# jhamrick/gaussian_processes

Measured on AMD Instinct MI355X. Metric: GP fit+predict wall-clock (kernel build + Cholesky + solve + log_lh + posterior mean), lower is better.
Workload: dtype f64; 1 GPU; N=65536 d=32 RBF(GaussianKernel) f64, m=1000 test points, h=1 w=0.5*sqrt(d) s=1; N=65536, d=32, m=1000, parallelism=1 GPU

## Files before the change

gaussian_processes_amd/_lib.py:

```python
import ctypes
import os
from ctypes import (POINTER, c_char_p, c_double, c_float, c_int, c_int64, c_size_t,
                    c_uint64, c_void_p)

import numpy as np

_HERE = os.path.dirname(os.path.abspath(__file__))
LIB_PATH = os.path.join(_HERE, "libgpx.so")

OK = 0
ERR_ARG, ERR_HIP, ERR_NO_DEVICE, ERR_NOMEM, ERR_UNSUPPORTED, ERR_INTERNAL = -1, -2, -3, -4, -5, -6
(ROUTE_TRSV_OPS, ROUTE_TRSV_STEPS, ROUTE_PANEL_RES, ROUTE_PANEL_CHAIN, ROUTE_FIT_RIDE, ROUTE_FIT_TWO_SOLVES,
 ROUTE_GEMM_FAST, ROUTE_GEMM_GENERIC, ROUTE_SYRK_EXACT, ROUTE_SYRK_PATCH, ROUTE_MG_BCAST_ONE, ROUTE_MG_BCAST_SAG,
 ROUTE_FIT_OPS_AHEAD, ROUTE_TRSM_OPS, ROUTE_POTRF_PAIR, ROUTE_VAR_CHUNK, ROUTE_LOO_CHUNK, ROUTE_TRSM_L_OPS,
 ROUTE_GRAD_CHUNK, ROUTE_EXTEND, ROUTE_SAMPLE, ROUTE_KAPPLY_FUSED, ROUTE_KAPPLY_GEMM, ROUTE_PATHS_GRAD_CHUNK) = range(24)
PROF_RANDN, PROF_RFF, PROF_KAPPLY, PROF_KAPPLY_GRAD = 14, 15, 16, 17
F64, F32 = 0, 1
KERNEL_GAUSSIAN, KERNEL_PERIODIC, KERNEL_GAUSSIAN_ARD = 0, 1, 2
ARD_MAX_D = 64
FULL, LOWER = 0, 1
(K, DK_DH, DK_DW, DK_DP, D2K_DHDH, D2K_DHDW, D2K_DHDP, D2K_DWDW, D2K_DWDP, D2K_DPDP) = range(10)
MIN_LOG = -705.6238298100243

MEMBER_BY_NAME = {
    "K": K, "dK_dh": DK_DH, "dK_dw": DK_DW, "dK_dp": DK_DP,
    "d2K_dhdh": D2K_DHDH, "d2K_dhdw": D2K_DHDW, "d2K_dwdh": D2K_DHDW,
    "d2K_dhdp": D2K_DHDP, "d2K_dpdh": D2K_DHDP, "d2K_dwdw": D2K_DWDW,
    "d2K_dwdp": D2K_DWDP, "d2K_dpdw": D2K_DWDP, "d2K_dpdp": D2K_DPDP,
}

# ... 103 lines not shown
    "gpx_gp_extend_from_K": (c_int, [c_void_p, c_double_p, c_double_p, c_int64, c_double_p, c_double_p, POINTER(c_void_p),
                                     c_int_p]),
    "gpx_gp_sample": (c_int, [c_void_p, c_double_p, c_int64, c_int64, c_uint64, c_int, c_double, c_double_p, c_int_p]),
    "gpx_gp_sample_from_K": (c_int, [c_void_p, c_double_p, c_double_p, c_int64, c_int64, c_uint64, c_int, c_double, c_double_p,
                                     c_int_p]),
    "gpx_gp_paths_create": (c_int, [c_void_p, c_int64, c_int64, c_uint64, POINTER(c_void_p)]),
    "gpx_paths_eval": (c_int, [c_void_p, c_double_p, c_int64, c_int64, c_double_p]),
    "gpx_paths_grad": (c_int, [c_void_p, c_double_p, c_int64, c_int64, c_double_p, c_double_p]),
    "gpx_paths_get": (c_int, [c_void_p, c_double_p, c_double_p, c_double_p]),
    "gpx_paths_describe": (c_int, [c_void_p, c_int_p, c_int_p, POINTER(c_int64), c_int_p, POINTER(c_int64), POINTER(c_int64),
                                   POINTER(c_uint64)]),
    "gpx_debug_paths_timing": (c_int, [c_void_p, POINTER(c_float)]),
    "gpx_paths_destroy": (c_int, [c_void_p]),
    "gpx_debug_var_plan": (c_int, [c_int, c_int64, c_int64, c_int64, c_size_t, POINTER(c_int64), POINTER(c_int64),
                                   POINTER(c_size_t)]),
    "gpx_gp_get_Kxx": (c_int, [c_void_p, c_double_p, c_int64]),
    "gpx_gp_get_Lxx": (c_int, [c_void_p, c_double_p, c_int64]),
    "gpx_gp_get_alpha": (c_int, [c_void_p, c_double_p]),
    "gpx_gp_get_inv_Kxx": (c_int, [c_void_p, c_double_p, c_int64]),
    "gpx_gp_dloglh_dtheta": (c_int, [c_void_p, c_double_p]),
    "gpx_gp_dlh_d2lh": (c_int, [c_void_p, c_double_p, c_double_p, c_double_p]),
    "gpx_gp_dm_dtheta": (c_int, [c_void_p, c_double_p, c_int64, c_double_p]),
    "gpx_gp_fit_batch": (c_int, [c_void_p, c_double_p, c_int64, c_double_p, c_int_p]),
    "gpx_gp_fit_batch_grad": (c_int, [c_void_p, c_double_p, c_int64, c_double_p, c_double_p, c_double_p, c_int_p]),
    "gpx_gp_save": (c_int, [c_void_p, c_char_p]),
    "gpx_gp_load": (c_int, [POINTER(c_void_p), c_char_p]),
    "gpx_gp_describe": (c_int, [c_void_p, c_int_p, c_int_p, POINTER(c_int64), c_int_p, c_double_p, c_double_p]),
    "gpx_gp_get_xy": (c_int, [c_void_p, c_double_p, c_double_p]),
    "gpx_gp_last_timing": (c_int, [c_void_p, POINTER(c_float)]),
    "gpx_gp_device_ptrs": (c_int, [c_void_p, POINTER(c_void_p), POINTER(c_int64), POINTER(c_void_p),
# ... 131 lines not shown
def mem_free():
    f, t = c_size_t(0), c_size_t(0)
    check(load().gpx_mem_info(ctypes.byref(f), ctypes.byref(t)))
    return int(f.value)


def var_plan(dtype_id, n, m, chunk_rows=0, free_bytes=None):
    if free_bytes is None:
        free_bytes = mem_free()
    rows, chunks, nbytes = c_int64(0), c_int64(0), c_size_t(0)
    check(load().gpx_debug_var_plan(int(dtype_id), int(n), int(m), int(chunk_rows), int(free_bytes), ctypes.byref(rows),
                                    ctypes.byref(chunks), ctypes.byref(nbytes)))
    return rows.value, chunks.value, int(nbytes.value)


def route_count(route):
    v = c_int64(0)
    check(load().gpx_debug_route_count(int(route), ctypes.byref(v)))
    return v.value


def route_reset():
    check(load().gpx_debug_route_reset())


def kapply_fused_max(value=-1):
    prev = c_int64(0)
    check(load().gpx_debug_kapply_fused_max(int(value), ctypes.byref(prev)))
    return prev.value

# ... 7 lines not shown
```

gaussian_processes_amd/csrc/gpx_common.h:

```cpp
#pragma once
#include <hip/hip_runtime.h>
#include <stdint.h>
#include <stdio.h>
#include <stdlib.h>
#include <string.h>
#include <math.h>
#include <vector>

#include "../../include/gpx.h"
#include "gpx_tune.h"

namespace gpx {

void set_error(const char *fmt, ...);
int  hip_fail(hipError_t e, const char *what, const char *file, int line);
int  ensure_device();

#define GPX_HIP(call)                                                        \
    do {                                                                     \
        hipError_t e__ = (call);                                             \
        if (e__ != hipSuccess) return gpx::hip_fail(e__, #call, __FILE__, __LINE__); \
    } while (0)

#define GPX_TRY(call)                                                        \
// ... 5 lines not shown
#define GPX_ARG(cond, msg)                                                   \
    do {                                                                     \
        if (!(cond)) { gpx::set_error("%s: %s", __func__, msg); return GPX_ERR_ARG; } \
    } while (0)

#define GPX_LAUNCH_CHECK()                                                   \
    do {                                                                     \
        hipError_t e__ = hipGetLastError();                                  \
        if (e__ != hipSuccess) return gpx::hip_fail(e__, "kernel launch", __FILE__, __LINE__); \
    } while (0)


enum Route { RT_TRSV_OPS = 0, RT_TRSV_STEPS = 1, RT_PANEL_RES = 2, RT_PANEL_CHAIN = 3, RT_FIT_RIDE = 4,
             RT_FIT_TWO_SOLVES = 5, RT_GEMM_FAST = 6, RT_GEMM_GENERIC = 7, RT_SYRK_EXACT = 8, RT_SYRK_PATCH = 9,
             RT_MG_BCAST_ONE = 10, RT_MG_BCAST_SAG = 11, RT_FIT_OPS_AHEAD = 12, RT_TRSM_OPS = 13, RT_POTRF_PAIR = 14, RT_VAR_CHUNK = 15, RT_LOO_CHUNK = 16,
             RT_TRSM_L_OPS = 17, RT_GRAD_CHUNK = 18, RT_EXTEND = 19, RT_SAMPLE = 20, RT_KAPPLY_FUSED = 21, RT_KAPPLY_GEMM = 22, RT_PATHS_GRAD_CHUNK = 23, RT_COUNT = 24 };
void route_hit(int route);

int check_internal_info(int info);

static inline hipStream_t S(void *s) { return (hipStream_t)s; }
static inline size_t esize(int dtype) { return dtype == GPX_F64 ? 8 : 4; }
static inline int64_t round_up(int64_t v, int64_t m) { return (v + m - 1) / m * m; }
static inline int64_t cdiv(int64_t a, int64_t b) { return (a + b - 1) / b; }

static inline int order(hipEvent_t e, hipStream_t from, hipStream_t to)
{
    GPX_HIP(hipEventRecord(e, from));
    GPX_HIP(hipStreamWaitEvent(to, e, 0));
    return GPX_OK;
}
struct EventPool {
// ... 96 lines not shown
constexpr int TRSV_OPS_BLOCK = 512;
static inline int64_t trsv_ops_nblocks(int64_t n) { return n / TRSV_OPS_BLOCK; }
static inline bool trsv_ops_whole_blocks(int64_t n) { return n >= TRSV_OPS_BLOCK && n % TRSV_OPS_BLOCK == 0; }
struct TrsvOps {
    GrowBuf mem;
    bool valid = false;
    int64_t built = 0;
    void invalidate() { valid = false; built = 0; }
    static TrsvOps view(void *p, size_t bytes) { TrsvOps o; o.mem.p = p; o.mem.bytes = bytes; return o; }
};
int trsv_ops_build(int dtype, const void *L, int64_t n, int64_t ldl, TrsvOps *ops, hipStream_t st);
bool trsv_ops_ahead_ok(int dtype, const void *L, int64_t n, int64_t ldl);
bool trsm_ops_ok(int dtype, const void *L, int64_t n, int64_t ldl);
size_t trsv_ops_bytes(int dtype, int64_t n);
int trsv_ops_build_upto(int dtype, const void *L, int64_t n, int64_t ldl, TrsvOps *ops, int64_t kend, hipStream_t st);
int trsv_lower(int dtype, const void *L, int64_t n, int64_t ldl, void *b, void *x, int transpose,
               hipStream_t st, const Batch *bt = nullptr,
               TrsvOps *ops = nullptr);
int trsm_right_lt(int dtype, const void *L, int64_t n, int64_t ldl, void *X, int64_t m, int64_t ldx,
                  hipStream_t st, int x_upper = 0, TrsvOps *ops = nullptr,
                  int64_t c0 = 0);
int trsm_right_l(int dtype, const void *L, int64_t n, int64_t ldl, void *X, int64_t m, int64_t ldx, hipStream_t st,
                 TrsvOps *ops = nullptr);
int pred_grad(int dtype, int kernel, const void *xo, int64_t m, const void *x, int64_t n, int d, const double *params,
              const void *alpha, const void *B, int64_t ldb, double scale, const double *col_div, double *out_dev, hipStream_t st);
int inv_from_factor(int dtype, const void *L, int64_t n, int64_t ldl, void *X, void *W, int tri, hipStream_t st,
                    TrsvOps *ops, int count = 1, int64_t sL = 0, void *group_ops = nullptr);
int logdet_chol(int dtype, const void *L, int64_t n, int64_t ldl, double *out_dev, hipStream_t st, int count = 1,
                int64_t sL = 0, int64_t so = 0);
int dot(int dtype, const void *a, const void *b, int64_t n, double *out_dev, hipStream_t st, int count = 1,
        int64_t sa = 0, int64_t sb = 0, int64_t so = 0);
int tril(int dtype, void *A, int64_t n, int64_t lda, hipStream_t st);
int var_rows(int dtype, int kernel, const void *X, int64_t rows, int64_t n, int64_t ldx, const void *xo, int d,
// ... 41 lines not shown
```

gaussian_processes_amd/csrc/gpx_gp.hip:

```cpp
#include "gpx_common.h"
#include <cmath>
#include <vector>

#include "gpx_gp_internal.h"

namespace gpx {

template <typename T>
__global__ void cvt_from_f64_2d(const double *__restrict__ src, int64_t lds, T *__restrict__ dst, int64_t ldd, int64_t rows, int64_t cols)
{
    const int64_t c = (int64_t)blockIdx.x * blockDim.x + threadIdx.x;
    if (c >= cols) return;
    for (int64_t r = blockIdx.y; r < rows; r += gridDim.y) dst[r * ldd + c] = (T)src[r * lds + c];
}

template <typename T>
__global__ void cvt_to_f64_2d(const T *__restrict__ src, int64_t lds, double *__restrict__ dst,
                              int64_t ldd, int64_t rows, int64_t cols, int lower_only)
{
    const int64_t c = (int64_t)blockIdx.x * blockDim.x + threadIdx.x;
    if (c >= cols) return;
    for (int64_t r = blockIdx.y; r < rows; r += gridDim.y) {
        const double v = (double)src[r * lds + c];
        dst[r * ldd + c] = (lower_only && c > r) ? 0.0 : v;
// ... 76 lines not shown
{
    GpScal sc;
    GPX_TRY(gp_read_scal(g, &sc));
    if (sc.info != 0) { set_error("Kxx is not positive definite (info = %d): there is no factor %s", sc.info, what_for); return GPX_ERR_ARG; }
    return GPX_OK;
}

int check_internal_info(int info)
{
    if (info >= 0) return GPX_OK;
    set_error("internal failure inside the factorisation (info = %d: a hand-off between workgroups of the resident "
              "panel kernel timed out); the factor is not valid -- this is NOT a statement about the matrix", info);
    return GPX_ERR_INTERNAL;
}

int gp_finish_fit(gpx_gp *g, bool rhs_is_row_n, int *info)
{
    const size_t es = esize(g->dtype);
    hipStream_t st = g->st;
    if (rhs_is_row_n) {
        GPX_TRY(trsv_lower(g->dtype, g->A, g->n, g->lda, (char *)g->A + (size_t)g->n * g->lda * es, g->alpha, 1, st, nullptr, &g->ops));
    } else {
        GPX_HIP(hipMemcpyAsync(g->t0, g->y, (size_t)g->n * es, hipMemcpyDeviceToDevice, st));
        GPX_TRY(trsv_lower(g->dtype, g->A, g->n, g->lda, g->t0, g->t1, 0, st, nullptr, &g->ops));
        GPX_TRY(trsv_lower(g->dtype, g->A, g->n, g->lda, g->t1, g->alpha, 1, st, nullptr, &g->ops));
    }
    GPX_HIP(hipEventRecord(g->ev[3], st));
    GPX_TRY(logdet_chol(g->dtype, g->A, g->n, g->lda, &g->scal->logdet, st));
    GPX_TRY(dot(g->dtype, g->y, g->alpha, g->n, &g->scal->yta, st));
    GPX_HIP(hipEventRecord(g->ev[4], st));
    g->fitted = true;
    if (info) {
        GPX_HIP(hipMemcpyAsync(info, &g->scal->info, sizeof(int), hipMemcpyDeviceToHost, st));
        GPX_HIP(hipStreamSynchronize(st));
        GPX_TRY(check_internal_info(*info));
    }
    return GPX_OK;
}

// ... 242 lines not shown
    GPX_ARG(cap >= 0 && (cap == 0 || params), "bad arguments");
    if (count) *count = g->nparams;
    for (int i = 0; i < g->nparams && i < cap; ++i) params[i] = g->params[i];
    return GPX_OK;
}

int gpx_gp_set_K(gpx_gp_t *g, const double *Kxx, int64_t ld)
{
    GP_ENTER(g);
    GPX_ARG(g && Kxx && ld >= g->n, "bad arguments");
    GPX_TRY(upload_f64(g->dtype, g->A, g->lda, Kxx, ld, g->n, g->n, g->st));
    g->have_K = true; gp_unfit(g);
    return GPX_OK;
}

struct OpsAhead { gpx_gp *g; int64_t group, last; };
static int ops_ahead_step(void *user, int64_t cols_done, hipEvent_t panel_done)
{
    OpsAhead *o = (OpsAhead *)user;
    gpx_gp *g = o->g;
    const int64_t ready = std::min(trsv_ops_nblocks(cols_done), o->last);
    if (ready - g->ops.built < o->group) return GPX_OK;
    GPX_HIP(hipStreamWaitEvent(g->st_ops, panel_done, 0));
    return trsv_ops_build_upto(g->dtype, g->A, g->n, g->lda, &g->ops, ready, g->st_ops);
}

int gpx_gp_fit(gpx_gp_t *g, int *info)
{
    GP_ENTER(g);
    GPX_ARG(g, "gp is NULL");
    GPX_ARG(g->have_data && (g->have_params || g->have_K),
            "set_data and set_params (or set_K) must be called before fit");
    const GpView v = gp_view(g);
    if (!g->have_K && (!g->x_finite || !kernel_values_finite(v.kernel, v.params, g->s, g->dtype))) {
        set_error("%s (%s)", NONFINITE_MSG, g->x_finite ? "kernel parameters or s" : "x");
        return GPX_ERR_ARG;
    }
    const size_t es = esize(g->dtype);
    hipStream_t st = g->st;
    GPX_HIP(hipEventRecord(g->ev[0], st));
    if (!g->have_K)
        GPX_TRY(kmat(g->dtype, v.kernel, GPX_K, v.x, g->n, v.x, g->n, g->d, v.params, g->s * g->s,
                     GPX_LOWER, g->A, g->lda, st));
    g->have_K = false;
    g->have_kii = false;
    GPX_HIP(hipEventRecord(g->ev[1], st));
    const int64_t ride_max = tune().fit_ride_max;
    const bool ride = g->n <= ride_max;
    route_hit(ride ? RT_FIT_RIDE : RT_FIT_TWO_SOLVES);
    if (ride) GPX_HIP(hipMemcpyAsync((char *)g->A + (size_t)g->n * g->lda * es, g->y, (size_t)g->n * es, hipMemcpyDeviceToDevice, st));
    g->ops.invalidate();
    const bool ahead = tune().fit_ops_ahead != 0 && g->n >= tune().fit_ops_ahead_min &&
                       trsv_ops_ahead_ok(g->dtype, g->A, g->n, g->lda);
    const int64_t nfull = trsv_ops_nblocks(g->n), tail = tune().fit_ops_tail;
    const int64_t group = std::max<int64_t>(1, std::min(nfull, nfull - tail));
    OpsAhead oa = {g, group, std::max<int64_t>(0, nfull - tail)};
    PotrfHook hook = {ops_ahead_step, &oa};
    if (ahead) {
        if (!g->st_ops) {
            int least = 0, greatest = 0;
            GPX_HIP(hipDeviceGetStreamPriorityRange(&least, &greatest));
            GPX_HIP(hipStreamCreateWithPriority(&g->st_ops, hipStreamNonBlocking, least));
            GPX_HIP(hipEventCreateWithFlags(&g->ev_ops, hipEventDisableTiming));
        }
        GPX_TRY(g->ops.mem.reserve(trsv_ops_bytes(g->dtype, g->n), st));
        GPX_TRY(order(g->ev_ops, st, g->st_ops));
    }
    GPX_TRY(potrf(g->dtype, g->A, g->n, g->lda, &g->scal->info, st, nullptr, ride ? 1 : 0, true, ahead ? &hook : nullptr));
    if (ahead) {
        GPX_TRY(order(g->ev_ops, g->st_ops, st));
        if (g->ops.built > 0) route_hit(RT_FIT_OPS_AHEAD);
    }
    GPX_HIP(hipEventRecord(g->ev[2], st));
    return gp_finish_fit(g, ride, info);
}

static int gp_scalars(gpx_gp_t *g, double *logdet, double *yta, int *info)
{
    GP_ENTER(g);
    GPX_ARG(g && g->fitted, "gp is not fitted");
    GpScal sc;
    GPX_TRY(gp_read_scal(g, &sc));
    if (logdet) *logdet = sc.logdet;
    if (yta) *yta = sc.yta;
    if (info) *info = sc.info;
    return GPX_OK;
}

int gpx_gp_log_lh(gpx_gp_t *g, double *log_lh)
// ... 296 lines not shown
    if (!g->have_kii) GPX_TRY(gp_loo_sweep(g, ch, dm, dv, dl));
    else GPX_TRY(loo_points(g->dtype, g->kii, g->y, g->alpha, n, dm, dv, dl, g->st));
    GPX_TRY(sum_f64(dl, n, ds, g->st));
    if (mean) GPX_HIP(hipMemcpyAsync(mean, dm, (size_t)n * sizeof(double), hipMemcpyDeviceToHost, g->st));
    if (var) GPX_HIP(hipMemcpyAsync(var, dv, (size_t)n * sizeof(double), hipMemcpyDeviceToHost, g->st));
    if (log_p) GPX_HIP(hipMemcpyAsync(log_p, dl, (size_t)n * sizeof(double), hipMemcpyDeviceToHost, g->st));
    if (log_p_sum) GPX_HIP(hipMemcpyAsync(log_p_sum, ds, sizeof(double), hipMemcpyDeviceToHost, g->st));
    GPX_HIP(hipStreamSynchronize(g->st));
    return GPX_OK;
}

int gpx_debug_var_plan(int dtype, int64_t n, int64_t m, int64_t chunk_rows, size_t free_bytes,
                       int64_t *rows_per_chunk, int64_t *chunks, size_t *bytes_per_chunk)
{
    return var_plan(dtype, n, m, chunk_rows, free_bytes, rows_per_chunk, chunks, bytes_per_chunk);
}

int gpx_gp_get_Kxx(gpx_gp_t *g, double *out, int64_t ld)
{
    GP_ENTER(g);
    GPX_ARG(g && g->have_data && g->have_params && out && ld >= g->n, "bad arguments");
    const size_t es = esize(g->dtype);
    DevBuf K;
    GPX_TRY(K.alloc((size_t)g->n * g->lda * es));
    const GpView v = gp_view(g);
    GPX_TRY(kmat(g->dtype, v.kernel, GPX_K, v.x, g->n, v.x, g->n, g->d, v.params, g->s * g->s,
                 GPX_FULL, K.p, g->lda, g->st));
    return download_f64(g->dtype, out, ld, K.p, g->lda, g->n, g->n, 0, g->st);
}

// ... 402 lines not shown
```

gaussian_processes_amd/csrc/gpx_gp_internal.h:

```cpp
#pragma once
#include "gpx_common.h"
#include <cstddef>

struct GpScal {
    double logdet;
    double yta;
    int x_bad, y_bad;
    int info;
    int pad;
};
static_assert(sizeof(GpScal) == 32 && offsetof(GpScal, x_bad) == 16 && offsetof(GpScal, info) == 24, "GpScal layout");

struct gpx_gp {
    int device;
    int dtype, kernel, d, nparams;
    int64_t n, lda;
    void *x, *y, *A, *alpha, *t0, *t1;
    void *xs;
    GpScal *scal;
    hipStream_t st;
    hipEvent_t ev[6];
    double params[1 + GPX_ARD_MAX_D];
    double iso[2];
    double s;
// ... 6 lines not shown
    double *kii;
    bool have_kii;
    hipStream_t st_ops;
    hipEvent_t ev_ops;
};

namespace gpx {
int gp_scan_finite(gpx_gp *g);
int upload_f64(int dtype, void *dst, int64_t ldd, const double *src, int64_t lds, int64_t rows, int64_t cols, hipStream_t st,
               DevBuf *stage = nullptr);
int download_f64(int dtype, double *dst, int64_t ldh, const void *src, int64_t lds, int64_t rows, int64_t cols, int lower_only,
                 hipStream_t st);
int gp_read_scal(gpx_gp *g, GpScal *host);
int gp_need_factor(gpx_gp *g, const char *what_for);
static inline void gp_unfit(gpx_gp *g) { g->fitted = false; g->have_kii = false; }
int gp_finish_fit(gpx_gp *g, bool rhs_is_row_n, int *info);
static inline int nparams_of(int kernel, int d) { return kernel == GPX_KERNEL_GAUSSIAN_ARD ? 1 + d : (kernel == GPX_KERNEL_PERIODIC ? 3 : 2); }
struct GpView { int kernel; const void *x; const double *params; };
static inline GpView gp_view(const gpx_gp *g)
{
    if (g->kernel == GPX_KERNEL_GAUSSIAN_ARD) return {GPX_KERNEL_GAUSSIAN, g->xs, g->iso};
    return {g->kernel, g->x, g->params};
}
int gp_rescale(gpx_gp *g);
}

#define GP_ENTER(g)                                                          \
    GPX_ARG((g) != nullptr, "gp is NULL");                                   \
    gpx::tune_refresh();                                                     \
    gpx::DeviceGuard guard__((g)->device);                                   \
    if (guard__.rc != GPX_OK) return guard__.rc;                             \
// ... 4 lines not shown
```

gaussian_processes_amd/csrc/gpx_runtime.hip:

```cpp
#include "gpx_common.h"
#include <stdarg.h>
#include <stddef.h>
#include <dlfcn.h>
#include <atomic>
#include <mutex>
#include <set>
#include <utility>
#include <vector>

namespace gpx {

static thread_local char g_err[512] = "";

void set_error(const char *fmt, ...)
{
    va_list ap;
    va_start(ap, fmt);
    vsnprintf(g_err, sizeof(g_err), fmt, ap);
    va_end(ap);
}

int hip_fail(hipError_t e, const char *what, const char *file, int line)
{
    set_error("HIP error %d (%s) in %s at %s:%d", (int)e, hipGetErrorString(e), what, file, line);
// ... 127 lines not shown
    }
    if (b) (void)hipEventRecord(b, st);
}

static void prof_clear()
{
    std::lock_guard<std::mutex> lk(g_prof_mu);
    for (auto &r : g_prof) {
        if (r.a) (void)hipEventDestroy(r.a);
        if (r.b) (void)hipEventDestroy(r.b);
    }
    g_prof.clear();
}

static std::atomic<long long> g_route[RT_COUNT];
void route_hit(int route) { if (route >= 0 && route < RT_COUNT) g_route[route].fetch_add(1, std::memory_order_relaxed); }

static std::mutex g_attr_mu;
static std::set<std::pair<const void *, int>> g_attr_done;

int set_max_lds(const void *fn, int bytes)
{
    int dev = 0;
    GPX_HIP(hipGetDevice(&dev));
    std::lock_guard<std::mutex> lk(g_attr_mu);
    const auto key = std::make_pair(fn, dev);
    if (g_attr_done.count(key)) return GPX_OK;
    GPX_HIP(hipFuncSetAttribute(fn, hipFuncAttributeMaxDynamicSharedMemorySize, bytes));
    g_attr_done.insert(key);
    return GPX_OK;
}
// ... 330 lines not shown
```

gaussian_processes_amd/csrc/gpx_solve.hip:

```cpp
#include "gpx_common.h"
#include "gpx_kernels_dev.h"
#include "gpx_leaf.h"

namespace gpx {

constexpr int SB = 64;
constexpr int OB = TRSV_OPS_BLOCK;

template <typename T>
__global__ __launch_bounds__(256) void inv64_kernel(const T *__restrict__ L, int64_t ldl, int64_t ncols,
                                                    T *__restrict__ out, int transposed, T *__restrict__ W,
                                                    T *__restrict__ Wt, int64_t bsL, int64_t bsOut)
{
    L += (int64_t)blockIdx.y * bsL;
    const int tid = threadIdx.x, tr = tid >> 4, tc = tid & 15;
    const int64_t k0 = (int64_t)blockIdx.x * SB;
    const int jb = (int)min((int64_t)SB, ncols - k0);
    const T *blk = L + k0 * ldl + k0;
    T a[4][4], x[4][4];
#pragma unroll
    for (int r = 0; r < 4; ++r)
#pragma unroll
        for (int c = 0; c < 4; ++c) {
            const int row = 4 * tr + r, col = 4 * tc + c;
// ... 475 lines not shown
        GPX_TRY(gemm_nt(dtype, OB, rag, OB, V.Wt(nfull - 1), OB, L + nfull * OB * ldl + (nfull - 1) * OB, ldl, tb, OB,
                        1.0, GPX_FULL, 0, 0, st, 1, 0));
    }
    return GPX_OK;
}

static bool ops_usable(int dtype, const void *L, int64_t ldl)
{
    static_assert(16 % (2 * sizeof(double)) == 0 && 16 % (2 * sizeof(float)) == 0, "16 is a multiple of 2 es");
    static_assert((16 / sizeof(double)) % 2 == 0 && (16 / sizeof(float)) % 2 == 0, "16 / es is even");
    return tune().trsv_ops != 0 && ((uintptr_t)L) % 16 == 0 && ldl % (16 / (int64_t)esize(dtype)) == 0;
}
static int64_t trsv_ops_min_n() { return std::max<int64_t>(2 * OB, tune().trsv_ops_min); }
bool trsv_ops_ahead_ok(int dtype, const void *L, int64_t n, int64_t ldl) { return n >= 2 * OB && trsv_ops_whole_blocks(n) && ops_usable(dtype, L, ldl); }
bool trsm_ops_ok(int dtype, const void *L, int64_t n, int64_t ldl) { return trsv_ops_ahead_ok(dtype, L, n, ldl) && tune().trsm_ops != 0; }

template <typename T>
struct Sweep {
    const T *L; int64_t n, ldl, ncols; T *b, *x; hipStream_t st;
    unsigned nbt; int64_t sL, sv;
    T *Linv; int64_t sLinv;
    int aligned;
    int64_t nb() const { return cdiv(ncols, TB); }
    int width(int64_t blk) const { return (int)std::min<int64_t>(TB, ncols - blk * TB); }
};

template <typename T>
static void inv64_blocks(const Sweep<T> &S, int64_t first, int transposed)
{
    hipLaunchKernelGGL((inv64_kernel<T>), dim3((unsigned)(cdiv(S.ncols, SB) - first), S.nbt), dim3(256), 0, S.st,
// ... 25 lines not shown
    for (int64_t blk = nb - 1; blk >= kfirst; --blk) {
        const int64_t k0 = blk * TB, q0 = k0 + TB;
        const int jb = S.width(blk), qjb = blk + 1 < nb ? S.width(blk + 1) : 0;
        if (qjb > 0)
            hipLaunchKernelGGL((trsv_bwd_fused<T, 32>), dim3((unsigned)(1 + cdiv(jb, 32)), S.nbt), dim3(TBT), 0, S.st, S.L,
                               S.ldl, S.Linv, S.b, S.x, k0, 0, q0, qjb, k0, k0 + jb, S.aligned, S.sL, S.sLinv, S.sv);
        hipLaunchKernelGGL((trsv_bwd_fused<T, 128>), dim3((unsigned)(1 + (qjb > 0 ? cdiv(k0, 128) : 0)), S.nbt),
                           dim3(TBT), 0, S.st, S.L, S.ldl, S.Linv, S.b, S.x, k0, jb, q0, qjb, (int64_t)0, k0, S.aligned,
                           S.sL, S.sLinv, S.sv);
    }
}

constexpr int NCH = OB / (TBT / OPL);

template <typename T>
static void ops_fwd(const Sweep<T> &S, const OpsView<T> &V)
{
    for (int64_t k = 0; k < V.nfull; ++k) {
        const int64_t k0 = k * OB, far0 = k0 + OB;
        const int64_t nfar = k > 0 ? cdiv(S.n - far0, 64) : 0;
        hipLaunchKernelGGL((trsv_op_kernel<T, true>), dim3((unsigned)(NCH + nfar)), dim3(TBT), 0, S.st, V.W(k),
                           k > 0 ? V.Tf(k) : (const T *)nullptr, S.L, S.ldl, S.b, S.x, S.n, k0, k0 - OB, k > 0 ? OB : 0, far0, S.n, NCH, 1);
    }
}

template <typename T>
static void ops_bwd(const Sweep<T> &S, const OpsView<T> &V, int64_t kend)
{
    for (int64_t k = kend - 1; k >= 0; --k) {
        const int64_t k0 = k * OB, q0 = k0 + OB;
        const int qjb = (k + 1 < V.nfull) ? OB : (int)(S.n - q0);
        const int64_t nfar = qjb > 0 ? cdiv(k0, 128) : 0;
        hipLaunchKernelGGL((trsv_op_kernel<T, false>), dim3((unsigned)(NCH + nfar)), dim3(TBT), 0, S.st, V.Wt(k),
                           qjb > 0 ? V.Tb(k) : (const T *)nullptr, S.L, S.ldl, S.b, S.x, S.n, k0, q0, qjb, (int64_t)0, k0, NCH, 1);
    }
}

template <typename T>
static int trsv_t(const T *L, int64_t n, int64_t ldl, T *b, T *x, int transpose, hipStream_t st,
                  int64_t ncols = -1, const Batch *bt = nullptr, TrsvOps *ops = nullptr)
{
    constexpr int dtype = sizeof(T) == 8 ? GPX_F64 : GPX_F32;
    if (ncols < 0 || ncols > n) ncols = n;
    Sweep<T> S;
    S.L = L; S.n = n; S.ldl = ldl; S.ncols = ncols; S.b = b; S.x = x; S.st = st;
    S.nbt = (unsigned)(bt ? bt->count : 1); S.sL = bt ? bt->sA : 0; S.sv = bt ? bt->sB : 0;
    ProfScope prof(PC_TRSV, ((double)n * ncols - 0.5 * (double)ncols * (ncols - 1)) * sizeof(T) * S.nbt, st);
    S.sLinv = cdiv(ncols, SB) * SB * SB;
    void *scr = nullptr;
    GPX_TRY(g_scr.get((size_t)S.nbt * S.sLinv * sizeof(T), &scr));
    S.Linv = (T *)scr;
    S.aligned = (((uintptr_t)L) % (2 * sizeof(T)) == 0) && (ldl % 2 == 0);
    const bool usable = !bt && ncols == n && ops_usable(dtype, L, ldl);
    const bool cached = ops && ops->mem.p && n % OB == 0 && ops->mem.bytes >= trsv_ops_bytes(dtype, n);
    const bool prebuilt = cached && ops->valid;
// ... 2 lines not shown
        route_hit(RT_TRSV_OPS);
        void *buf = nullptr;
        if (ops) {
            bool grew = false;
            GPX_TRY(ops->mem.reserve(trsv_ops_bytes(dtype, n), st, &grew));
            if (grew) ops->invalidate();
            buf = ops->mem.p;
        } else {
            GPX_TRY(g_ops.get(trsv_ops_bytes(dtype, n), &buf));
        }
        const OpsView<T> V(buf, n);
        if (!ops || !ops->valid) GPX_TRY(trsv_ops_prepare<T>(L, n, ldl, buf, st, ops ? std::min(ops->built, V.nfull) : 0, V.nfull));
        if (ops) { ops->valid = true; ops->built = V.nfull; }
        const bool ragged = n > V.nfull * OB;
        if (!transpose) {
            ops_fwd(S, V);
            if (ragged) { inv64_blocks(S, 0, 1); steps_fwd(S, V.nfull); }
        } else {
            if (ragged) { inv64_blocks(S, 0, 0); steps_bwd(S, V.nfull); }
            ops_bwd(S, V, V.nfull);
        }
    } else if (!transpose) {
        route_hit(RT_TRSV_STEPS);
        inv64_blocks(S, 0, 1);
        steps_fwd(S, 0);
    } else {
        route_hit(RT_TRSV_STEPS);
        inv64_blocks(S, kpart * (OB / SB), 0);
        steps_bwd(S, kpart);
        if (kpart > 0) {
            route_hit(RT_TRSV_OPS);
            ops_bwd(S, OpsView<T>(ops->mem.p, n), kpart);
        }
    }
    GPX_LAUNCH_CHECK();
    return GPX_OK;
}

int trsv_lower(int dtype, const void *L, int64_t n, int64_t ldl, void *b, void *x, int transpose,
               hipStream_t st, const Batch *bt, TrsvOps *ops)
{
    if (n <= 0) return GPX_OK;
    if (dtype == GPX_F64)
        return trsv_t<double>((const double *)L, n, ldl, (double *)b, (double *)x, transpose, st, -1, bt, ops);
    return trsv_t<float>((const float *)L, n, ldl, (float *)b, (float *)x, transpose, st, -1, bt, ops);
}

int trsv_ops_build(int dtype, const void *L, int64_t n, int64_t ldl, TrsvOps *ops, hipStream_t st)
{
    if (!ops || !trsv_ops_whole_blocks(n) || !ops_usable(dtype, L, ldl)) return GPX_OK;
    GPX_TRY(ops->mem.reserve(trsv_ops_bytes(dtype, n), st));
    ops->invalidate();
    if (dtype == GPX_F64) GPX_TRY(trsv_ops_prepare<double>((const double *)L, n, ldl, ops->mem.p, st));
    else GPX_TRY(trsv_ops_prepare<float>((const float *)L, n, ldl, ops->mem.p, st));
    ops->valid = true;
    ops->built = n / OB;
    return GPX_OK;
}

int trsv_ops_build_upto(int dtype, const void *L, int64_t n, int64_t ldl, TrsvOps *ops, int64_t kend, hipStream_t st)
// ... 702 lines not shown
```

gaussian_processes_amd/csrc/gpx_tune.h:

```cpp
#pragma once
#include <stdint.h>

namespace gpx {

#define GPX_TUNE_LIST(X, XF, XS, X2)                                                                                   \
                                                                               \
    XF(gemm_no_fast, "GPX_GEMM_NO_FAST")                                                                               \
    X(gemm_ablate, "GPX_GEMM_ABLATE", 0)                                                                               \
    X(gemm_pad_lds, "GPX_GEMM_PAD_LDS", 0)                                                                             \
    X(gemm_bn64_tiles, "GPX_GEMM_BN64_TILES", 256)                                                                     \
    X(gemm_exact, "GPX_GEMM_EXACT", 1)                                                                                 \
    X(gemm_fine_tiles, "GPX_GEMM_FINE_TILES", 16384)                                                                   \
    X2(syrk_bn64_tiles, "GPX_SYRK_BN64_TILES", 2600, 4000)                                                             \
                                                              \
    X(fit_ride_max, "GPX_FIT_RIDE_MAX", 16384)                                                                         \
    X(fit_ops_ahead, "GPX_FIT_OPS_AHEAD", 1)                                                                           \
    X(fit_ops_ahead_min, "GPX_FIT_OPS_AHEAD_MIN", 8192)                                                                \
    X(fit_ops_tail, "GPX_FIT_OPS_TAIL", 4)                                                                             \
    XS(batch_max, "GPX_BATCH_MAX", 1)                                                                                  \
    X(io_block_bytes, "GPX_IO_BLOCK_BYTES", (int64_t)64 << 20)                                                         \
    X(kmat_panel_bytes, "GPX_KMAT_PANEL_BYTES", (int64_t)256 << 20)                                                    \
                                                                        \
    XF(force_collectives, "GPX_FORCE_COLLECTIVES")                                                                     \
    X(mg_bcast_chunks, "GPX_MG_BCAST_CHUNKS", 4)                                                                       \
    XF(mg_no_timing, "GPX_MG_NO_TIMING")                                                                               \
    XS(mg_owner_first, "GPX_MG_OWNER_FIRST", 0)                                                                        \
                                                                  \
    XF(trace, "GPX_TRACE")                                                                                             \
    X(potrf_res, "GPX_POTRF_RES", 256)                                                                                 \
    X(res_strict, "GPX_RES_STRICT", 1)                                                                                 \
    X(two_part_rows, "GPX_POTRF_TWO_PART_ROWS", 16384)                                                                 \
// ... 49 lines not shown
```

include/gpx.h:

```cpp
#ifndef GPX_H
#define GPX_H

#include <stddef.h>
#include <stdint.h>

#ifdef __cplusplus
extern "C" {
#endif

#define GPX_VERSION 100

#define GPX_OK              0
#define GPX_ERR_ARG        -1
#define GPX_ERR_HIP        -2
#define GPX_ERR_NO_DEVICE  -3
#define GPX_ERR_NOMEM      -4
#define GPX_ERR_UNSUPPORTED -5
#define GPX_ERR_INTERNAL   -6

#define GPX_F64 0
#define GPX_F32 1

#define GPX_KERNEL_GAUSSIAN 0
#define GPX_KERNEL_PERIODIC 1
// ... 80 lines not shown
#define GPX_ROUTE_SYRK_PATCH      9
#define GPX_ROUTE_MG_BCAST_ONE   10
#define GPX_ROUTE_MG_BCAST_SAG   11
#define GPX_ROUTE_FIT_OPS_AHEAD  12
#define GPX_ROUTE_TRSM_OPS       13
#define GPX_ROUTE_POTRF_PAIR     14
#define GPX_ROUTE_VAR_CHUNK      15
#define GPX_ROUTE_LOO_CHUNK      16
#define GPX_ROUTE_TRSM_L_OPS     17
#define GPX_ROUTE_GRAD_CHUNK     18
#define GPX_ROUTE_EXTEND         19
#define GPX_ROUTE_SAMPLE         20
#define GPX_ROUTE_KAPPLY_FUSED   21
#define GPX_ROUTE_KAPPLY_GEMM    22
#define GPX_ROUTE_PATHS_GRAD_CHUNK 23
int gpx_debug_route_count(int route, int64_t *count);
int gpx_debug_roctx_ranges(int64_t *count);
int gpx_debug_route_reset(void);
int gpx_debug_tune_refreshes(int64_t *count);
int gpx_debug_kapply_fused_max(int64_t value, int64_t *previous);
int gpx_debug_leaf_selfcheck(int run_now, int *state);


int gpx_d_kmat(int dtype, int kernel, int member, const void *x1, int64_t n,
               const void *x2, int64_t m, int d, const double *params,
               double diag_add, int tri, void *out, int64_t ld, void *stream);

int gpx_d_scale_points(int dtype, const void *x, int64_t n, int d, const double *w_host, void *out, void *stream);

int gpx_d_mean(int dtype, int kernel, const void *xo, int64_t m, const void *x,
// ... 81 lines not shown
int gpx_gp_get_params(gpx_gp_t *gp, double *params, int cap, int *count);
int gpx_gp_set_K(gpx_gp_t *gp, const double *Kxx, int64_t ld);
int gpx_gp_fit(gpx_gp_t *gp, int *info);
int gpx_gp_log_lh(gpx_gp_t *gp, double *log_lh);
int gpx_gp_logdet(gpx_gp_t *gp, double *logdet);
int gpx_gp_info(gpx_gp_t *gp, int *info);
int gpx_gp_mean(gpx_gp_t *gp, const double *xo, int64_t m, double *out);
int gpx_gp_cov(gpx_gp_t *gp, const double *xo, int64_t m, double *out);
int gpx_gp_mean_from_K(gpx_gp_t *gp, const double *Kxox, int64_t m, double *out);
int gpx_gp_cov_from_K(gpx_gp_t *gp, const double *Kxox, const double *Kxoxo, int64_t m,
                      double *out);
int gpx_gp_var(gpx_gp_t *gp, const double *xo, int64_t m, int64_t chunk_rows, double *out);
int gpx_gp_var_from_K(gpx_gp_t *gp, const double *Kxox, const double *kdiag, int64_t m, int64_t chunk_rows, double *out);
int gpx_debug_var_plan(int dtype, int64_t n, int64_t m, int64_t chunk_rows, size_t free_bytes,
                       int64_t *rows_per_chunk, int64_t *chunks, size_t *bytes_per_chunk);
int gpx_gp_inv_diag(gpx_gp_t *gp, int64_t chunk_rows, double *out);
int gpx_gp_loo(gpx_gp_t *gp, int64_t chunk_rows, double *mean, double *var, double *log_p, double *log_p_sum);
int gpx_gp_mean_grad(gpx_gp_t *gp, const double *xo, int64_t m, double *grad);
int gpx_gp_var_grad(gpx_gp_t *gp, const double *xo, int64_t m, int64_t chunk_rows, double *var, double *grad);
int gpx_gp_extend(gpx_gp_t *gp, const double *x_new, const double *y_new, int64_t k, gpx_gp_t **out, int *info);
int gpx_gp_extend_from_K(gpx_gp_t *gp, const double *x_new, const double *y_new, int64_t k,
                         const double *Knew_old, const double *Knew_new, gpx_gp_t **out, int *info);
int gpx_gp_sample(gpx_gp_t *gp, const double *xo, int64_t m, int64_t S, uint64_t seed, int noise, double jitter,
                  double *out , int *info);
int gpx_gp_sample_from_K(gpx_gp_t *gp, const double *Kxox, const double *Kxoxo, int64_t m, int64_t S, uint64_t seed,
                         int noise, double jitter, double *out, int *info);
int gpx_gp_get_Kxx(gpx_gp_t *gp, double *out, int64_t ld);
int gpx_gp_get_Lxx(gpx_gp_t *gp, double *out, int64_t ld);
int gpx_gp_get_alpha(gpx_gp_t *gp, double *out);
int gpx_gp_get_inv_Kxx(gpx_gp_t *gp, double *out, int64_t ld);
// ... 97 lines not shown
```

Before: 1.343 s.

## Sweep forward triangular solve on side stream while Cholesky factorization proceeds

When the fit does not ride the RHS in the factor (N above fit_ride_max), the forward substitution L t1 = y now runs on the ops stream for leading blocks whose inverse operators are already built, interleaved with the ongoing potrf panels. The operator build is also regrouped into halving batches so forward sweeps can start earlier, and the final forward solve resumes from the first unswept block. This overlaps the latency-bound trsv with the factorization, at the cost of contention with potrf on the GPU and more side-stream launches. The feature is enabled by default by changing fit_ops_ahead to 3.

```diff
diff --git a/gaussian_processes_amd/_lib.py b/gaussian_processes_amd/_lib.py
--- a/gaussian_processes_amd/_lib.py
+++ b/gaussian_processes_amd/_lib.py
@@ -13,7 +13,7 @@
 (ROUTE_TRSV_OPS, ROUTE_TRSV_STEPS, ROUTE_PANEL_RES, ROUTE_PANEL_CHAIN, ROUTE_FIT_RIDE, ROUTE_FIT_TWO_SOLVES,
  ROUTE_GEMM_FAST, ROUTE_GEMM_GENERIC, ROUTE_SYRK_EXACT, ROUTE_SYRK_PATCH, ROUTE_MG_BCAST_ONE, ROUTE_MG_BCAST_SAG,
  ROUTE_FIT_OPS_AHEAD, ROUTE_TRSM_OPS, ROUTE_POTRF_PAIR, ROUTE_VAR_CHUNK, ROUTE_LOO_CHUNK, ROUTE_TRSM_L_OPS,
- ROUTE_GRAD_CHUNK, ROUTE_EXTEND, ROUTE_SAMPLE, ROUTE_KAPPLY_FUSED, ROUTE_KAPPLY_GEMM, ROUTE_PATHS_GRAD_CHUNK) = range(24)
+ ROUTE_GRAD_CHUNK, ROUTE_EXTEND, ROUTE_SAMPLE, ROUTE_KAPPLY_FUSED, ROUTE_KAPPLY_GEMM, ROUTE_PATHS_GRAD_CHUNK, ROUTE_FIT_FWD_AHEAD) = range(25)
 PROF_RANDN, PROF_RFF, PROF_KAPPLY, PROF_KAPPLY_GRAD = 14, 15, 16, 17
 F64, F32 = 0, 1
 KERNEL_GAUSSIAN, KERNEL_PERIODIC, KERNEL_GAUSSIAN_ARD = 0, 1, 2
@@ -147,6 +147,7 @@
     "gpx_paths_destroy": (c_int, [c_void_p]),
     "gpx_debug_var_plan": (c_int, [c_int, c_int64, c_int64, c_int64, c_size_t, POINTER(c_int64), POINTER(c_int64),
                                    POINTER(c_size_t)]),
+    "gpx_debug_fit_ops_plan": (c_int, [c_int64, c_int64, c_int64, c_int64, POINTER(c_int64)]),
     "gpx_gp_get_Kxx": (c_int, [c_void_p, c_double_p, c_int64]),
     "gpx_gp_get_Lxx": (c_int, [c_void_p, c_double_p, c_int64]),
     "gpx_gp_get_alpha": (c_int, [c_void_p, c_double_p]),
@@ -308,6 +309,12 @@
     return rows.value, chunks.value, int(nbytes.value)
 
 
+def fit_ops_plan(n, block, tail, cols_done):
+    k = c_int64(0)
+    check(load().gpx_debug_fit_ops_plan(int(n), int(block), int(tail), int(cols_done), ctypes.byref(k)))
+    return k.value
+
+
 def route_count(route):
     v = c_int64(0)
     check(load().gpx_debug_route_count(int(route), ctypes.byref(v)))
diff --git a/gaussian_processes_amd/csrc/gpx_common.h b/gaussian_processes_amd/csrc/gpx_common.h
--- a/gaussian_processes_amd/csrc/gpx_common.h
+++ b/gaussian_processes_amd/csrc/gpx_common.h
@@ -43,8 +43,10 @@
 enum Route { RT_TRSV_OPS = 0, RT_TRSV_STEPS = 1, RT_PANEL_RES = 2, RT_PANEL_CHAIN = 3, RT_FIT_RIDE = 4,
              RT_FIT_TWO_SOLVES = 5, RT_GEMM_FAST = 6, RT_GEMM_GENERIC = 7, RT_SYRK_EXACT = 8, RT_SYRK_PATCH = 9,
              RT_MG_BCAST_ONE = 10, RT_MG_BCAST_SAG = 11, RT_FIT_OPS_AHEAD = 12, RT_TRSM_OPS = 13, RT_POTRF_PAIR = 14, RT_VAR_CHUNK = 15, RT_LOO_CHUNK = 16,
-             RT_TRSM_L_OPS = 17, RT_GRAD_CHUNK = 18, RT_EXTEND = 19, RT_SAMPLE = 20, RT_KAPPLY_FUSED = 21, RT_KAPPLY_GEMM = 22, RT_PATHS_GRAD_CHUNK = 23, RT_COUNT = 24 };
-void route_hit(int route);
+             RT_TRSM_L_OPS = 17, RT_GRAD_CHUNK = 18, RT_EXTEND = 19, RT_SAMPLE = 20, RT_KAPPLY_FUSED = 21, RT_KAPPLY_GEMM = 22, RT_PATHS_GRAD_CHUNK = 23,
+             RT_FIT_FWD_AHEAD = 24,
+             RT_COUNT = 25 };
+void route_hit(int route, long long times = 1);
 
 int check_internal_info(int info);
 
@@ -171,9 +173,13 @@
 bool trsm_ops_ok(int dtype, const void *L, int64_t n, int64_t ldl);
 size_t trsv_ops_bytes(int dtype, int64_t n);
 int trsv_ops_build_upto(int dtype, const void *L, int64_t n, int64_t ldl, TrsvOps *ops, int64_t kend, hipStream_t st);
+bool trsv_ops_fwd_ahead_ok(int dtype, const void *L, int64_t n, int64_t ldl);
+int trsv_ops_fwd_range(int dtype, const void *L, int64_t n, int64_t ldl, const TrsvOps *ops, void *b, void *x, int64_t kbeg, int64_t kend,
+                       hipStream_t st);
 int trsv_lower(int dtype, const void *L, int64_t n, int64_t ldl, void *b, void *x, int transpose,
                hipStream_t st, const Batch *bt = nullptr,
-               TrsvOps *ops = nullptr);
+               TrsvOps *ops = nullptr,
+               int64_t kfirst = 0);
 int trsm_right_lt(int dtype, const void *L, int64_t n, int64_t ldl, void *X, int64_t m, int64_t ldx,
                   hipStream_t st, int x_upper = 0, TrsvOps *ops = nullptr,
                   int64_t c0 = 0);
diff --git a/gaussian_processes_amd/csrc/gpx_gp.hip b/gaussian_processes_amd/csrc/gpx_gp.hip
--- a/gaussian_processes_amd/csrc/gpx_gp.hip
+++ b/gaussian_processes_amd/csrc/gpx_gp.hip
@@ -114,15 +114,15 @@
     return GPX_ERR_INTERNAL;
 }
 
-int gp_finish_fit(gpx_gp *g, bool rhs_is_row_n, int *info)
+int gp_finish_fit(gpx_gp *g, bool rhs_is_row_n, int *info, int64_t fwd_done)
 {
     const size_t es = esize(g->dtype);
     hipStream_t st = g->st;
     if (rhs_is_row_n) {
         GPX_TRY(trsv_lower(g->dtype, g->A, g->n, g->lda, (char *)g->A + (size_t)g->n * g->lda * es, g->alpha, 1, st, nullptr, &g->ops));
     } else {
-        GPX_HIP(hipMemcpyAsync(g->t0, g->y, (size_t)g->n * es, hipMemcpyDeviceToDevice, st));
-        GPX_TRY(trsv_lower(g->dtype, g->A, g->n, g->lda, g->t0, g->t1, 0, st, nullptr, &g->ops));
+        if (fwd_done == 0) GPX_HIP(hipMemcpyAsync(g->t0, g->y, (size_t)g->n * es, hipMemcpyDeviceToDevice, st));
+        GPX_TRY(trsv_lower(g->dtype, g->A, g->n, g->lda, g->t0, g->t1, 0, st, nullptr, &g->ops, fwd_done));
         GPX_TRY(trsv_lower(g->dtype, g->A, g->n, g->lda, g->t1, g->alpha, 1, st, nullptr, &g->ops));
     }
     GPX_HIP(hipEventRecord(g->ev[3], st));
@@ -395,15 +395,35 @@
     return GPX_OK;
 }
 
-struct OpsAhead { gpx_gp *g; int64_t group, last; };
+int64_t fit_ops_plan(int64_t n, int64_t block, int64_t tail, bool several, int64_t cols_done)
+{
+    const int64_t nfull = n / block, last = nfull - std::min(nfull, std::max<int64_t>(tail, 0));
+    const int64_t ready = std::min(std::min(cols_done, n) / block, last);
+    if (!several) return ready == last ? last : 0;
+    int64_t due = 0;
+    while (due < last) {
+        const int64_t next = std::min(last, due + (nfull - due + 1) / 2);
+        if (next > ready) break;
+        due = next;
+    }
+    return due;
+}
+
+struct OpsAhead { gpx_gp *g; int64_t tail; bool fwd; int64_t swept; };
 static int ops_ahead_step(void *user, int64_t cols_done, hipEvent_t panel_done)
 {
     OpsAhead *o = (OpsAhead *)user;
     gpx_gp *g = o->g;
-    const int64_t ready = std::min(trsv_ops_nblocks(cols_done), o->last);
-    if (ready - g->ops.built < o->group) return GPX_OK;
+    const int64_t due = fit_ops_plan(g->n, TRSV_OPS_BLOCK, o->tail, o->fwd, cols_done);
+    if (due <= g->ops.built) return GPX_OK;
     GPX_HIP(hipStreamWaitEvent(g->st_ops, panel_done, 0));
-    return trsv_ops_build_upto(g->dtype, g->A, g->n, g->lda, &g->ops, ready, g->st_ops);
+    GPX_TRY(trsv_ops_build_upto(g->dtype, g->A, g->n, g->lda, &g->ops, due, g->st_ops));
+    if (o->fwd && g->ops.built == due) {
+        GPX_TRY(trsv_ops_fwd_range(g->dtype, g->A, g->n, g->lda, &g->ops, g->t0, g->t1, o->swept, due, g->st_ops));
+        route_hit(RT_FIT_FWD_AHEAD, due - o->swept);
+        o->swept = due;
+    }
+    return GPX_OK;
 }
 
 int gpx_gp_fit(gpx_gp_t *g, int *info)
@@ -431,11 +451,10 @@
     route_hit(ride ? RT_FIT_RIDE : RT_FIT_TWO_SOLVES);
     if (ride) GPX_HIP(hipMemcpyAsync((char *)g->A + (size_t)g->n * g->lda * es, g->y, (size_t)g->n * es, hipMemcpyDeviceToDevice, st));
     g->ops.invalidate();
-    const bool ahead = tune().fit_ops_ahead != 0 && g->n >= tune().fit_ops_ahead_min &&
-                       trsv_ops_ahead_ok(g->dtype, g->A, g->n, g->lda);
-    const int64_t nfull = trsv_ops_nblocks(g->n), tail = tune().fit_ops_tail;
-    const int64_t group = std::max<int64_t>(1, std::min(nfull, nfull - tail));
-    OpsAhead oa = {g, group, std::max<int64_t>(0, nfull - tail)};
+    const int64_t bits = tune().fit_ops_ahead;
+    const bool ahead = (bits & 1) != 0 && g->n >= tune().fit_ops_ahead_min && trsv_ops_ahead_ok(g->dtype, g->A, g->n, g->lda);
+    const bool fwd_ahead = ahead && !ride && (bits & 2) != 0 && trsv_ops_fwd_ahead_ok(g->dtype, g->A, g->n, g->lda);
+    OpsAhead oa = {g, tune().fit_ops_tail, fwd_ahead, 0};
     PotrfHook hook = {ops_ahead_step, &oa};
     if (ahead) {
         if (!g->st_ops) {
@@ -445,6 +464,7 @@
             GPX_HIP(hipEventCreateWithFlags(&g->ev_ops, hipEventDisableTiming));
         }
         GPX_TRY(g->ops.mem.reserve(trsv_ops_bytes(g->dtype, g->n), st));
+        if (fwd_ahead) GPX_HIP(hipMemcpyAsync(g->t0, g->y, (size_t)g->n * es, hipMemcpyDeviceToDevice, st));
         GPX_TRY(order(g->ev_ops, st, g->st_ops));
     }
     GPX_TRY(potrf(g->dtype, g->A, g->n, g->lda, &g->scal->info, st, nullptr, ride ? 1 : 0, true, ahead ? &hook : nullptr));
@@ -453,7 +473,7 @@
         if (g->ops.built > 0) route_hit(RT_FIT_OPS_AHEAD);
     }
     GPX_HIP(hipEventRecord(g->ev[2], st));
-    return gp_finish_fit(g, ride, info);
+    return gp_finish_fit(g, ride, info, oa.swept);
 }
 
 static int gp_scalars(gpx_gp_t *g, double *logdet, double *yta, int *info)
@@ -780,6 +800,14 @@
                        int64_t *rows_per_chunk, int64_t *chunks, size_t *bytes_per_chunk)
 {
     return var_plan(dtype, n, m, chunk_rows, free_bytes, rows_per_chunk, chunks, bytes_per_chunk);
+}
+
+int gpx_debug_fit_ops_plan(int64_t n, int64_t block, int64_t tail, int64_t cols_done, int64_t *blocks_due)
+{
+    tune_refresh();
+    GPX_ARG(n >= 0 && block >= 1 && cols_done >= 0 && blocks_due, "bad arguments");
+    *blocks_due = fit_ops_plan(n, block, tail, n > tune().fit_ride_max && (tune().fit_ops_ahead & 2) != 0, cols_done);
+    return GPX_OK;
 }
 
 int gpx_gp_get_Kxx(gpx_gp_t *g, double *out, int64_t ld)
diff --git a/gaussian_processes_amd/csrc/gpx_gp_internal.h b/gaussian_processes_amd/csrc/gpx_gp_internal.h
--- a/gaussian_processes_amd/csrc/gpx_gp_internal.h
+++ b/gaussian_processes_amd/csrc/gpx_gp_internal.h
@@ -44,7 +44,7 @@
 int gp_read_scal(gpx_gp *g, GpScal *host);
 int gp_need_factor(gpx_gp *g, const char *what_for);
 static inline void gp_unfit(gpx_gp *g) { g->fitted = false; g->have_kii = false; }
-int gp_finish_fit(gpx_gp *g, bool rhs_is_row_n, int *info);
+int gp_finish_fit(gpx_gp *g, bool rhs_is_row_n, int *info, int64_t fwd_done = 0);
 static inline int nparams_of(int kernel, int d) { return kernel == GPX_KERNEL_GAUSSIAN_ARD ? 1 + d : (kernel == GPX_KERNEL_PERIODIC ? 3 : 2); }
 struct GpView { int kernel; const void *x; const double *params; };
 static inline GpView gp_view(const gpx_gp *g)
diff --git a/gaussian_processes_amd/csrc/gpx_runtime.hip b/gaussian_processes_amd/csrc/gpx_runtime.hip
--- a/gaussian_processes_amd/csrc/gpx_runtime.hip
+++ b/gaussian_processes_amd/csrc/gpx_runtime.hip
@@ -165,7 +165,7 @@
 }
 
 static std::atomic<long long> g_route[RT_COUNT];
-void route_hit(int route) { if (route >= 0 && route < RT_COUNT) g_route[route].fetch_add(1, std::memory_order_relaxed); }
+void route_hit(int route, long long times) { if (route >= 0 && route < RT_COUNT) g_route[route].fetch_add(times, std::memory_order_relaxed); }
 
 static std::mutex g_attr_mu;
 static std::set<std::pair<const void *, int>> g_attr_done;
diff --git a/gaussian_processes_amd/csrc/gpx_solve.hip b/gaussian_processes_amd/csrc/gpx_solve.hip
--- a/gaussian_processes_amd/csrc/gpx_solve.hip
+++ b/gaussian_processes_amd/csrc/gpx_solve.hip
@@ -513,6 +513,7 @@
 static int64_t trsv_ops_min_n() { return std::max<int64_t>(2 * OB, tune().trsv_ops_min); }
 bool trsv_ops_ahead_ok(int dtype, const void *L, int64_t n, int64_t ldl) { return n >= 2 * OB && trsv_ops_whole_blocks(n) && ops_usable(dtype, L, ldl); }
 bool trsm_ops_ok(int dtype, const void *L, int64_t n, int64_t ldl) { return trsv_ops_ahead_ok(dtype, L, n, ldl) && tune().trsm_ops != 0; }
+bool trsv_ops_fwd_ahead_ok(int dtype, const void *L, int64_t n, int64_t ldl) { return trsv_ops_ahead_ok(dtype, L, n, ldl) && n >= trsv_ops_min_n(); }
 
 template <typename T>
 struct Sweep {
@@ -568,9 +569,9 @@
 constexpr int NCH = OB / (TBT / OPL);
 
 template <typename T>
-static void ops_fwd(const Sweep<T> &S, const OpsView<T> &V)
-{
-    for (int64_t k = 0; k < V.nfull; ++k) {
+static void ops_fwd(const Sweep<T> &S, const OpsView<T> &V, int64_t kbeg, int64_t kend)
+{
+    for (int64_t k = kbeg; k < kend; ++k) {
         const int64_t k0 = k * OB, far0 = k0 + OB;
         const int64_t nfar = k > 0 ? cdiv(S.n - far0, 64) : 0;
         hipLaunchKernelGGL((trsv_op_kernel<T, true>), dim3((unsigned)(NCH + nfar)), dim3(TBT), 0, S.st, V.W(k),
@@ -592,7 +593,7 @@
 
 template <typename T>
 static int trsv_t(const T *L, int64_t n, int64_t ldl, T *b, T *x, int transpose, hipStream_t st,
-                  int64_t ncols = -1, const Batch *bt = nullptr, TrsvOps *ops = nullptr)
+                  int64_t ncols = -1, const Batch *bt = nullptr, TrsvOps *ops = nullptr, int64_t kfirst = 0)
 {
     constexpr int dtype = sizeof(T) == 8 ? GPX_F64 : GPX_F32;
     if (ncols < 0 || ncols > n) ncols = n;
@@ -625,7 +626,7 @@
         if (ops) { ops->valid = true; ops->built = V.nfull; }
         const bool ragged = n > V.nfull * OB;
         if (!transpose) {
-            ops_fwd(S, V);
+            ops_fwd(S, V, kfirst, V.nfull);
             if (ragged) { inv64_blocks(S, 0, 1); steps_fwd(S, V.nfull); }
         } else {
             if (ragged) { inv64_blocks(S, 0, 0); steps_bwd(S, V.nfull); }
@@ -649,12 +650,38 @@
 }
 
 int trsv_lower(int dtype, const void *L, int64_t n, int64_t ldl, void *b, void *x, int transpose,
-               hipStream_t st, const Batch *bt, TrsvOps *ops)
+               hipStream_t st, const Batch *bt, TrsvOps *ops, int64_t kfirst)
 {
     if (n <= 0) return GPX_OK;
+    if (kfirst > 0 && (transpose || bt || !ops || !trsv_ops_fwd_ahead_ok(dtype, L, n, ldl) || kfirst > std::min(ops->built, n / OB))) {
+        set_error("trsv_lower: %lld leading blocks cannot have been swept ahead of this solve", (long long)kfirst);
+        return GPX_ERR_ARG;
+    }
     if (dtype == GPX_F64)
-        return trsv_t<double>((const double *)L, n, ldl, (double *)b, (double *)x, transpose, st, -1, bt, ops);
-    return trsv_t<float>((const float *)L, n, ldl, (float *)b, (float *)x, transpose, st, -1, bt, ops);
+        return trsv_t<double>((const double *)L, n, ldl, (double *)b, (double *)x, transpose, st, -1, bt, ops, kfirst);
+    return trsv_t<float>((const float *)L, n, ldl, (float *)b, (float *)x, transpose, st, -1, bt, ops, kfirst);
+}
+
+template <typename T>
+static void ops_fwd_range_t(const T *L, int64_t n, int64_t ldl, const void *buf, T *b, T *x, int64_t kbeg, int64_t kend, hipStream_t st)
+{
+    Sweep<T> S;
+    S.L = L; S.n = n; S.ldl = ldl; S.ncols = n; S.b = b; S.x = x; S.st = st;
+    S.nbt = 1; S.sL = 0; S.sv = 0; S.Linv = nullptr; S.sLinv = 0; S.aligned = 1;
+    ops_fwd(S, OpsView<T>(buf, n), kbeg, kend);
+}
+int trsv_ops_fwd_range(int dtype, const void *L, int64_t n, int64_t ldl, const TrsvOps *ops, void *b, void *x, int64_t kbeg, int64_t kend,
+                       hipStream_t st)
+{
+    if (kbeg >= kend) return GPX_OK;
+    if (!ops || !ops->mem.p || !trsv_ops_fwd_ahead_ok(dtype, L, n, ldl) || kbeg < 0 || kend > ops->built) {
+        set_error("trsv_ops_fwd_range: blocks [%lld, %lld) have no operators", (long long)kbeg, (long long)kend);
+        return GPX_ERR_ARG;
+    }
+    if (dtype == GPX_F64) ops_fwd_range_t<double>((const double *)L, n, ldl, ops->mem.p, (double *)b, (double *)x, kbeg, kend, st);
+    else ops_fwd_range_t<float>((const float *)L, n, ldl, ops->mem.p, (float *)b, (float *)x, kbeg, kend, st);
+    GPX_LAUNCH_CHECK();
+    return GPX_OK;
 }
 
 int trsv_ops_build(int dtype, const void *L, int64_t n, int64_t ldl, TrsvOps *ops, hipStream_t st)
diff --git a/gaussian_processes_amd/csrc/gpx_tune.h b/gaussian_processes_amd/csrc/gpx_tune.h
--- a/gaussian_processes_amd/csrc/gpx_tune.h
+++ b/gaussian_processes_amd/csrc/gpx_tune.h
@@ -14,7 +14,8 @@
     X2(syrk_bn64_tiles, "GPX_SYRK_BN64_TILES", 2600, 4000)                                                             \
                                                               \
     X(fit_ride_max, "GPX_FIT_RIDE_MAX", 16384)                                                                         \
-    X(fit_ops_ahead, "GPX_FIT_OPS_AHEAD", 1)                                                                           \
+       \
+    X(fit_ops_ahead, "GPX_FIT_OPS_AHEAD", 3)                                                                           \
     X(fit_ops_ahead_min, "GPX_FIT_OPS_AHEAD_MIN", 8192)                                                                \
     X(fit_ops_tail, "GPX_FIT_OPS_TAIL", 4)                                                                             \
     XS(batch_max, "GPX_BATCH_MAX", 1)                                                                                  \
diff --git a/include/gpx.h b/include/gpx.h
--- a/include/gpx.h
+++ b/include/gpx.h
@@ -118,6 +118,7 @@
 #define GPX_ROUTE_KAPPLY_FUSED   21
 #define GPX_ROUTE_KAPPLY_GEMM    22
 #define GPX_ROUTE_PATHS_GRAD_CHUNK 23
+#define GPX_ROUTE_FIT_FWD_AHEAD  24
 int gpx_debug_route_count(int route, int64_t *count);
 int gpx_debug_roctx_ranges(int64_t *count);
 int gpx_debug_route_reset(void);
@@ -229,6 +230,7 @@
 int gpx_gp_var_from_K(gpx_gp_t *gp, const double *Kxox, const double *kdiag, int64_t m, int64_t chunk_rows, double *out);
 int gpx_debug_var_plan(int dtype, int64_t n, int64_t m, int64_t chunk_rows, size_t free_bytes,
                        int64_t *rows_per_chunk, int64_t *chunks, size_t *bytes_per_chunk);
+int gpx_debug_fit_ops_plan(int64_t n, int64_t block, int64_t tail, int64_t cols_done, int64_t *blocks_due);
 int gpx_gp_inv_diag(gpx_gp_t *gp, int64_t chunk_rows, double *out);
 int gpx_gp_loo(gpx_gp_t *gp, int64_t chunk_rows, double *mean, double *var, double *log_p, double *log_p_sum);
 int gpx_gp_mean_grad(gpx_gp_t *gp, const double *xo, int64_t m, double *grad);
```

Result: no change. 1.340 s (median of 6 runs) (-0.2%).
